# shgaurav1/DVG

Hardware: AMD Instinct MI355X
Metric: predicted frames/sec at 64x64, batch 64, 10-in/10-out (higher is better)
Workload: dtype f32; 1 GPU; Moving-MNIST 64x64 rollout (generate_frames.py make_gifs sample loop), vgg_64 + lstm + GP trigger sample at i%15==0, batch 64 per GPU, 10-in/10-out; model_family=vgg, batch_per_gpu=64, n_past=10, n_future=10, parallelism=replicas x1 (no data-path collective), launch=hipGraph replay, rollouts_in_flight=3, tile_policy=energy, loop_invariant_skip_halves=hoisted, upsample_conv3x3=as transposed 4x4/s2 conv, conv3x3_deep_layers=Winograd F(4x4,3x3) / F(2x2,3x3)

## Files before the change

dvg_amd/_lib.py:

```python
from __future__ import annotations

import ctypes as C
import os
import threading

_HERE = os.path.dirname(os.path.abspath(__file__))
LIB_PATH = os.environ.get("DVG_HIP_LIB") or os.path.join(_HERE, "csrc", "libdvg_hip.so")

_p = C.c_void_p
_i = C.c_int
_f = C.c_float
_d = C.c_double
_l = C.c_long
_ip = C.POINTER(C.c_int)

SIGNATURES = {
    "dvg_abi_version": (_i, []),
    "dvg_last_error": (C.c_char_p, []),
    "dvg_stream_capture_id": (_l, [_p]),
    "dvg_mfma_mode": (_i, []),
    "dvg_build_info": (C.c_char_p, []),
    "dvg_set_tile_policy": (None, [_i]),
    "dvg_tile_policy": (_i, []),
    "dvg_packed_row_floats": (_i, []),
    "dvg_pack_conv_weight": (_i, [_p, _p, _i, _i, _i, _i, _p]),
    "dvg_pack_convT_weight": (_i, [_p, _p, _i, _i, _i, _i, _p]),
    "dvg_unpack_conv_weight": (_i, [_p, _p, _i, _i, _i, _i, _p]),
    "dvg_unpack_convT_weight": (_i, [_p, _p, _i, _i, _i, _i, _p]),
    "dvg_conv_first_stats_rows": (_i, [_i, _i, _i, _i]),
    "dvg_pack_conv_weight_k16": (_i, [_p, _p, _i, _i, _i, _i, _i, _p]),
    "dvg_conv_splitk_v2": (_i, [_i, _i, _i, _i, _i, _i]),
    "dvg_conv_stats_rows_v2": (_i, [_i, _i, _i, _i, _i, _i, _i, _i]),
    "dvg_conv3x3_bn_act_v2": (_i, [_p, _p, _p, _p, _p, _p, _p, _p, _i, _i, _i, _i, _i, _i, _i, _i, _f, _p, _l, _p, _p, _i, _p]),
    "dvg_conv3x3_first_pair": (_i, [_p, _p, _p, _p, _p, _p, _p, _p, _p, _i, _i, _i, _i, _i, _f, _i, _p]),
    "dvg_conv4x4s2_bn_act_v2": (_i, [_p, _p, _p, _p, _p, _p, _i, _i, _i, _i, _i, _i, _f, _p, _l, _p]),
    "dvg_convT4x4s2_bn_act_v2": (_i, [_p, _p, _p, _p, _p, _p, _p, _i, _i, _i, _i, _i, _i, _i, _f, _p, _l, _p, _p, _i, _p]),
    "dvg_convT4x4s2_bn_act_proj": (_i, [_p, _p, _p, _p, _p, _p, _i, _i, _i, _i, _i, _i, _i, _f, _p, _p, _i, _p]),
    "dvg_winograd_weight": (_i, [_p, _p, _i, _i, _i, _p]),
    "dvg_winograd_input": (_i, [_p, _p, _i, _i, _i, _i, _i, _i, _p]),
    "dvg_gemm_batched_k16": (_i, [_p, _p, _p, _i, _i, _i, _i, _i, _p]),
    "dvg_gemm_batched_plan": (_i, [_i, _i, _i, _i, _i, _ip, _ip, _ip]),
    "dvg_winograd_transform_width": (_i, [_l, _i]),
    "dvg_winograd_output": (_i, [_p, _p, _p, _p, _p, _i, _i, _i, _i, _i, _f, _i, _p, _i, _p]),
    "dvg_winograd_output_input": (_i, [_p, _p, _p, _p, _i, _i, _i, _i, _i, _f, _p, _p]),
    "dvg_stem_up_winograd_input": (_i, [_p, _i, _p, _i, _p, _p, _p, _i, _i, _i, _i, _f, _p]),
    "dvg_winograd_output_up_input": (_i, [_p, _p, _p, _p, _i, _i, _i, _i, _i, _f, _p]),
    "dvg_winograd_output_pool_input": (_i, [_p, _p, _p, _p, _p, _i, _i, _i, _i, _i, _f, _i, _p]),
    "dvg_conv3x3_first": (_i, [_p, _p, _p, _p, _p, _p, _i, _i, _i, _i, _i, _i, _f, _p]),
    "dvg_convT3x3_last": (_i, [_p, _p, _p, _p, _i, _i, _i, _i, _i, _i, _p]),
    "dvg_conv4x4s2_first": (_i, [_p, _p, _p, _p, _p, _p, _i, _i, _i, _i, _i, _i, _f, _p]),
    "dvg_convT4x4s2_last": (_i, [_p, _p, _p, _p, _p, _i, _i, _i, _i, _i, _i, _i, _p]),
    "dvg_moving_mnist_compose": (_i, [_p, _p, _p, _p, _i, _i, _i, _i, _i, _i, _p]),
    "dvg_clip_gather_u8": (_i, [_p, _p, _p, _l, _i, _i, _i, _i, _i, _i, _p]),
    "dvg_clip_gather_aug_u8": (_i, [_p, _p, _p, _p, _p, _l, _i, _i, _i, _i, _i, _i, _p]),
    "dvg_mnist_scale_u8": (_i, [_p, _p, _i, _i, _i, _p, _p, _p]),
    "dvg_moving_mnist_compose_u8": (_i, [_p, _p, _p, _p, _i, _i, _i, _i, _i, _i, _p]),
    "dvg_resample_u8_band": (_i, [_p, _i, _i, _i, _i, _i, _i, _p]),
    "dvg_resample_u8": (_i, [_p, _p, _i, _i, _i, _i, _i, _i, _p, _p, _i, _p, _p, _i, _p, _p]),
    "dvg_eval_frames": (_i, [_p, _p, _p, _p, _i, _i, _i, _p]),
    "dvg_eval_frames_finn": (_i, [_p, _p, _p, _p, _p, _i, _i, _i, _i, _p]),
    "dvg_pairwise_frame_mse": (_i, [_p, _p, _i, _l, _i, _l, _i, _p]),
    "dvg_frame_mosaic": (_i, [_p, _l, _p, _l, _p, _l, _i, _i, _i, _p] + [_i] * 9 + [_p, _i, _p, _i, _i, _p, _i, _i, _i, _i, _p, _p]),
    "dvg_adam_step": (_i, [_p, _p, _p, _p, _l, _f, _f, _f, _f, _f, _i, _p, _p]),
    "dvg_pixel_proj": (_i, [_p, _p, _p, _l, _i, _i, _p]),
    "dvg_convT_gather": (_i, [_p, _p, _p, _p, _i, _i, _i, _i, _i, _i, _p, _i, _p]),
    "dvg_channel_stats_rows": (_i, [_l]),
    "dvg_channel_stats": (_i, [_p, _p, _l, _i, _i, _p]),
    "dvg_bn_finalize": (_i, [_p, _i, _p, _p, _p, _p, _p, _p, _p, _p, _i, _d, _f, _f, _p, _i, _i, _p, _p]),
    "dvg_channel_stats_pivot": (_i, [_p, _p, _p, _l, _i, _i, _p]),
    "dvg_bn_finalize_pivot": (_i, [_p, _i, _p, _p, _p, _p, _p, _p, _p, _p, _p, _i, _d, _f, _f, _p, _i, _i, _p, _p]),
    "dvg_bn_running_update": (_i, [_p, _p, _i, _i, _f, _f, _f, _p, _p, _p, _i, _p]),
    "dvg_bn_act_apply": (_i, [_p, _p, _p, _p, _p, _i, _i, _i, _i, _i, _f, _i, _p]),
    "dvg_gemm_nt_bias_act": (_i, [_p, _p, _p, _p, _p, _p, _i, _i, _i, _i, _i, _i, _i, _i, _f, _i, _p]),
    "dvg_lstm_cell": (_i, [_p, _p, _p, _p, _p, _p, _p, _p, _p, _p, _i, _i, _p]),
    "dvg_lstm_cell_pre": (_i, [_p, _p, _p, _p, _p, _p, _p, _i, _i, _p]),
    "dvg_lstm_cell_bwd": (_i, [_p, _p, _p, _p, _p, _p, _p, _p, _p, _p, _i, _i, _p]),
    "dvg_lstm_cell_x": (_i, [_p, _i, _i, _p, _p, _p, _i, _p, _p, _p, _p, _i, _i, _p]),
    "dvg_gru_cell": (_i, [_p, _p, _p, _p, _p, _p, _p, _p, _i, _i, _p]),
    "dvg_gru_cell_pre": (_i, [_p, _p, _p, _p, _p, _p, _i, _i, _p]),
    "dvg_rnn_cell": (_i, [_p, _p, _p, _p, _p, _p, _p, _i, _i, _p]),
    "dvg_gru_gates_bwd": (_i, [_p, _p, _p, _p, _p, _p, _p, _i, _i, _p]),
    "dvg_stem_gemm": (_i, [_p, _i, _p, _i, _p, _p, _p, _i, _i, _i, _i, _i, _i, _f, _p]),
    "dvg_gp_precision": (_i, [_i, _i, _i]),
    "dvg_gp_bwd_precision": (_i, [_i, _i]),
    "dvg_gp_lds_bytes": (C.c_size_t, [_i, _i, _i]),
    "dvg_gp_predict": (_i, [_p] * 14 + [_i, _i, _i, _i, _f, _i, _i, _p]),
    "dvg_gp_step_group": (_i, [_i, _i, _i, _i]),
    "dvg_gp_bwd_lds_bytes": (C.c_size_t, [_i, _i]),
    "dvg_gp_bwd_chunk": (_i, [_i, _i]),
    "dvg_gemm_tn": (_i, [_p] * 5 + [_i] * 8 + [_p]),
    "dvg_gp_train_bwd": (_i, [_p] * 17 + [_i, _i, _i, _f, _i, _i, _p]),
    "dvg_sum_steps_multi": (_i, [_p, _p, _p, _i, _i, _p]),
    "dvg_gp_elbo": (_i, [_p, _p, _p, _p, _l, _l, _p, _p, _i, _i, _i, _i, _p]),
    "dvg_gp_elbo_bwd": (_i, [_p, _p, _p, _p, _l, _l, _p, _p, _p, _p, _p, _p, _p, _i, _i, _i, _i, _p]),
    "dvg_bn_act_bwd_rows": (_i, [_i, _i, _i, _i]),
    "dvg_bn_act_bwd_reduce": (_i, [_p, _p, _p, _p, _p, _p, _i, _i, _i, _i, _i, _f, _i, _p]),
    "dvg_bn_bwd_finalize": (_i, [_p, _i, _p, _p, _p, _p, _p, _p, _p, _p, _p, _i, _d, _i, _i, _i, _p]),
    "dvg_bn_act_bwd_reduce_centered": (_i, [_p, _p, _p, _p, _p, _p, _p, _i, _i, _i, _i, _i, _f, _i, _p]),
    "dvg_bn_bwd_finalize_centered": (_i, [_p, _i, _p, _p, _p, _p, _p, _p, _p, _p, _p, _i, _d, _i, _i, _i, _p]),
    "dvg_affine3_apply": (_i, [_p, _p, _p, _p, _p, _p, _l, _i, _p, _i, _i, _p]),
    "dvg_act_bwd": (_i, [_p, _p, _p, _l, _i, _f, _p]),
    "dvg_upsample2x_bwd": (_i, [_p, _p, _i, _i, _i, _i, _p]),
    "dvg_group_sum": (_i, [_p, _p, _p, _i, _i, _l, _p]),
    "dvg_colsum": (_i, [_p, _p, _i, _i, _i, _p]),
    "dvg_wgrad_finish": (_i, [_p, _i, _p, _i, _i, _i, _i, _i, _i, _i, _f, _p]),
    "dvg_k4_to_w3": (_i, [_p, _p, _i, _i, _i, _i, _f, _p]),
    "dvg_reduce_partials": (_i, [_p, _p, _i, _l, _p]),
    "dvg_conv_wgrad_splits": (_i, [_i, _i, _i, _i, _i, _i]),
    "dvg_conv_wgrad": (_i, [_i, _p, _p, _p, _p, _i, _i, _i, _i, _i, _i, _i, _p]),
    "dvg_conv_wgrad_splits_multi": (_i, [_i, _i, _i, _i, _i, _i, _i]),
    "dvg_conv_wgrad_multi": (_i, [_i, _i, _p, _p, _p, _p, _i, _i, _i, _i, _i, _i, _i, _p]),
    "dvg_winograd_wgrad_operands": (_i, [_p, _p, _p, _p, _i, _i, _i, _i, _i, _l, _l, _p]),
    "dvg_winograd_wgrad_splits": (_i, [_l, _i, _i]),
    "dvg_winograd_wgrad_gemm": (_i, [_p, _p, _p, _l, _i, _i, _p]),
    "dvg_winograd_wgrad_gemm_items": (_i, [_p, _p, _i, _l, _p, _i, _i, _p]),
    "dvg_winograd_wgrad_reduce": (_i, [_p, _i, _p, _i, _i, _p]),
    "dvg_wgrad_thin_rows": (_i, [_i, _i, _i, _i]),
    "dvg_wgrad_thin": (_i, [_p, _p, _p, _i, _i, _i, _i, _i, _i, _p]),
    "dvg_lstm_gates_bwd": (_i, [_p, _p, _p, _p, _p, _p, _p, _i, _i, _p]),
    "dvg_nchw_to_nhwc": (_i, [_p, _p, _i, _i, _i, _i, _p]),
    "dvg_nhwc_to_nchw": (_i, [_p, _p, _i, _i, _i, _i, _p]),
    "dvg_zero_tick": (_i, [_p, _l, _p, _p, _p, _p, _p]),
    "dvg_grad_sumsq_blocks": (_i, [_l]),
    "dvg_grad_sumsq": (_i, [_p, _l, _p, _p]),
    "dvg_grad_guard_finish": (_i, [_p, _i, _d, _i, _p, _p, _p]),
    "dvg_adam_step_guarded": (_i, [_p, _p, _p, _p, _l, _f, _f, _f, _f, _f, _i, _p, _p, _p, _p]),
    "dvg_ema_update_blocks": (_i, [_l]),
    "dvg_ema_update": (_i, [_p, _p, _l, _d, _p, _p, _p]),
    "dvg_lr_schedule_tick": (_i, [_i, _i, _i, _i, _d, _d, _p, _p, _p]),
    "dvg_adam_step_scheduled": (_i, [_p, _p, _p, _p, _l, _f, _f, _f, _f, _f, _i, _p, _p, _p, _p, _p]),
    "dvg_optim_step": (_i, [_i, _p, _p, _p, _p, _l, _f, _f, _f, _f, _f, _i, _p, _i, _p, _p, _p, _p, _p]),
    "dvg_val_accumulate": (_i, [_p, _p, _p, _i, _i, _i, _p, _p, _p, _p]),
    "dvg_frame_losses_blocks": (_i, [_l]),
    "dvg_frame_losses": (_i, [_p, _p, _p, _p, _l, _i, _i, _p, _p, _p]),
    "dvg_mse_sum_grad": (_i, [_p, _p, _p, _p, _l, _f, _p]),
    "dvg_frame_losses_ext_blocks": (_i, [_i, _l, _i, _i]),
    "dvg_frame_losses_ext": (_i, [_p, _p, _p, _p, _i, _i, _l, _i, _i, _i, _f, _p, _p, _p, _p]),
    "dvg_frame_ssim_loss_blocks": (_i, [_i, _l, _i, _i]),
    "dvg_frame_ssim_loss": (_i, [_p, _p, _p, _p, _i, _i, _l, _i, _i, _p, _i, _p, _p]),
    "dvg_gp_var_norms": (_i, [_p, _p, _i, _i, _p]),
    "dvg_gp_trigger_step": (_i, [_p, _i, _i, _i, _p, _i, _f, _p, _p, _p, _p, _i, _p]),
    "dvg_gp_trigger_replay": (_i, [_p, _i, _p, _i, _f, _p, _p, _p]),
    "dvg_gp_trigger_select": (_i, [_p, _p, _p, _p, _i, _i, _i, _l, _p, _p, _p, _p]),
    "dvg_debug_set_clockbuf": (None, [_p, C.c_uint]),
    "dvg_debug_set_gp_clockbuf": (None, [_p, C.c_uint]),
    "dvg_debug_set_wgrad_clockbuf": (None, [_p, C.c_uint]),
}

_lock = threading.Lock()
_lib = None


class DvgLibraryError(RuntimeError):
    pass


def lib() -> C.CDLL:
    global _lib
    if _lib is not None:
        return _lib
    with _lock:
        if _lib is not None:
            return _lib
        if not os.path.exists(LIB_PATH):
            raise DvgLibraryError(
                f"{LIB_PATH} not found: the HIP kernel library has not been built. "
                "Run `python -c 'import __graft_entry__ as g; g.build()'` (or `make -C dvg_amd/csrc`). "
                "There is no CPU/eager fallback for the DVG hot path.")
        try:
            import torch
            if torch.cuda.is_available():
                torch.cuda.init()
        except ImportError:
            pass
        try:
            handle = C.CDLL(LIB_PATH)
        except OSError as e:
            raise DvgLibraryError(f"cannot load {LIB_PATH}: {e}") from e
        for name, (res, args) in SIGNATURES.items():
            try:
                fn = getattr(handle, name)
            except AttributeError as e:
                raise DvgLibraryError(f"{LIB_PATH} lacks symbol {name}; rebuild it") from e
            fn.restype = res
            fn.argtypes = args
        _lib = handle
        return _lib


def build_info() -> dict:
    raw = lib().dvg_build_info().decode()
    d = {}
    for tok in raw.split():
        k, _, v = tok.partition("=")
        d[k] = int(v) if v.lstrip("-").isdigit() else v
# ... 13 lines not shown
```

dvg_amd/csrc/winograd.hip:

```cpp
#include <cstdlib>

#include "dvg_common.h"

namespace dvg {

__global__ void winograd_weight_kernel(const float* __restrict__ w, float* __restrict__ u, int cout, int cin) {
    const unsigned total = (unsigned)cout * (unsigned)cin / 2;
    for (unsigned i = blockIdx.x * blockDim.x + threadIdx.x; i < total; i += gridDim.x * blockDim.x) {
        const unsigned rr = i >> 3;
        const int co = (int)(rr % (unsigned)cout), chunk = (int)(rr / (unsigned)cout), k = (int)(i & 7) * 2;
        const float* g = w + ((size_t)co * cin + chunk * 16 + k) * 9;
        float t[2][4][3];
#pragma unroll
        for (int e = 0; e < 2; ++e)
#pragma unroll
            for (int s = 0; s < 3; ++s) {
                const float g0 = g[9 * e + s], g1 = g[9 * e + 3 + s], g2 = g[9 * e + 6 + s];
                t[e][0][s] = g0;
                t[e][1][s] = 0.5f * (g0 + g1 + g2);
                t[e][2][s] = 0.5f * (g0 - g1 + g2);
                t[e][3][s] = g2;
            }
        const unsigned row0 = ((unsigned)(co >> 6) * (unsigned)(cin / 16) + (unsigned)chunk) * 64u + (unsigned)(co & 63);
        const unsigned pos_rows = (unsigned)(cout >> 6) * (unsigned)(cin / 16) * 64u;
// ... 342 lines not shown
            for (int qq = 0; qq < 4; ++qq) {
                const float ad = addend ? addend[(((size_t)n * HW + 4 * ty + pp) * HW + 4 * tx + qq) * C + c] : 0.f;
                ys[((4 * ty + pp) * HW + 4 * tx + qq) * CS + cl] = apply_act((o[qq] + ad) * sc + sf, act, slope);
            }
        }
    }
    __syncthreads();
    float e[6][6];
#pragma unroll
    for (int b = 0; b < 6; ++b) {
        const int xx = 4 * tx - 1 + b;
        float d[6];
#pragma unroll
        for (int a = 0; a < 6; ++a) {
            const int yy = 4 * ty - 1 + a;
            d[a] = ((unsigned)yy < (unsigned)HW && (unsigned)xx < (unsigned)HW) ? ys[(yy * HW + xx) * CS + cl] : 0.f;
        }
        float col[6];
        bt4(d, col);
#pragma unroll
        for (int a = 0; a < 6; ++a) e[a][b] = col[a];
    }
#pragma unroll
    for (int a = 0; a < 6; ++a) {
        float o[6];
        bt4(e[a], o);
#pragma unroll
        for (int b = 0; b < 6; ++b) v[((size_t)(a * 6 + b) * T + t) * C + c] = o[b];
    }
}

template <int HW, int CS, typename V, bool POOL, int NT, bool UP = false>
__global__ __launch_bounds__(NT) void winograd4_chain_kernel(const float* __restrict__ m, const float* __restrict__ scale,
                                                             const float* __restrict__ shift, float* __restrict__ y,
                                                             float* __restrict__ v, int N, int C, int act, float slope,
                                                             const float* __restrict__ addend, int y_from) {
    constexpr int VN = VecN<V>::N;
    constexpr int WT = HW / 4, TI = WT * WT;
    static_assert(!(POOL && UP), "pool and upsample exclude each other");
    constexpr int SS = POOL ? HW / 2 : HW;
    constexpr int S2 = UP ? 2 * HW : SS;
    constexpr int WT2 = S2 / 4, TI2 = WT2 * WT2;
    constexpr int CV = CS / VN;
    extern __shared__ __attribute__((aligned(16))) float chain_ys[];
    float* const ys = chain_ys;
    const int cblocks = C / CS;
    const int n = blockIdx.x / cblocks, c0 = (blockIdx.x % cblocks) * CS;
    const int CVg = C / VN;
    const long T = (long)N * TI;
    for (int u = threadIdx.x; u < TI * CV; u += NT) {
        const int cv = u % CV, t_img = u / CV, ty = t_img / WT, tx = t_img % WT;
        const long t = (long)n * TI + t_img;
        const int cg = c0 / VN + cv;
        V s[4][6];
#pragma unroll
        for (int b = 0; b < 6; ++b) {
            V q[6];
#pragma unroll
            for (int a = 0; a < 6; ++a) q[a] = __builtin_nontemporal_load(reinterpret_cast<const V*>(m) + ((size_t)(a * 6 + b) * T + t) * CVg + cg);
            V col[4];
            at4(q, col);
#pragma unroll
            for (int pp = 0; pp < 4; ++pp) s[pp][b] = col[pp];
        }
        V sc, sf;
#pragma unroll
        for (int k = 0; k < VN; ++k) {
            vset(sc, k, scale ? scale[c0 + cv * VN + k] : 1.f);
            vset(sf, k, shift ? shift[c0 + cv * VN + k] : 0.f);
        }
        V val[4][4];
#pragma unroll
        for (int pp = 0; pp < 4; ++pp) {
            V o[4];
            at4(s[pp], o);
#pragma unroll
            for (int qq = 0; qq < 4; ++qq) {
                V ad = vzero<V>();
                if (addend) ad = reinterpret_cast<const V*>(addend)[(((size_t)n * HW + 4 * ty + pp) * HW + 4 * tx + qq) * CVg + cg];
#pragma unroll
                for (int k = 0; k < VN; ++k)
                    vset(val[pp][qq], k, apply_act((vget(o[qq], k) + vget(ad, k)) * vget(sc, k) + vget(sf, k), act, slope));
                if (POOL) {
                    if (n >= y_from)
                        reinterpret_cast<V*>(y)[(((size_t)(n - y_from) * HW + 4 * ty + pp) * HW + 4 * tx + qq) * CVg + cg] = val[pp][qq];
                } else
                    *reinterpret_cast<V*>(&ys[((4 * ty + pp) * HW + 4 * tx + qq) * CS + cv * VN]) = val[pp][qq];
            }
        }
        if (POOL) {
#pragma unroll
            for (int pp = 0; pp < 2; ++pp)
#pragma unroll
                for (int qq = 0; qq < 2; ++qq) {
                    V mx;
#pragma unroll
                    for (int k = 0; k < VN; ++k)
                        vset(mx, k, fmaxf(fmaxf(vget(val[2 * pp][2 * qq], k), vget(val[2 * pp][2 * qq + 1], k)),
                                          fmaxf(vget(val[2 * pp + 1][2 * qq], k), vget(val[2 * pp + 1][2 * qq + 1], k))));
                    *reinterpret_cast<V*>(&ys[((2 * ty + pp) * SS + 2 * tx + qq) * CS + cv * VN]) = mx;
                }
        }
    }
    __syncthreads();
    const long T2 = (long)N * TI2;
    for (int u = threadIdx.x; u < TI2 * CV; u += NT) {
        const int cv = u % CV, t_img = u / CV, ty = t_img / WT2, tx = t_img % WT2;
        const long t2 = (long)n * TI2 + t_img;
        const int cg = c0 / VN + cv;
        V e[6][6];
#pragma unroll
        for (int b = 0; b < 6; ++b) {
            const int xx = 4 * tx - 1 + b;
            V d[6];
#pragma unroll
            for (int a = 0; a < 6; ++a) {
                const int yy = 4 * ty - 1 + a;
                d[a] = ((unsigned)yy < (unsigned)S2 && (unsigned)xx < (unsigned)S2)
                           ? *reinterpret_cast<const V*>(&ys[((yy >> (UP ? 1 : 0)) * SS + (xx >> (UP ? 1 : 0))) * CS + cv * VN])
                           : vzero<V>();
            }
            V col[6];
            bt4(d, col);
#pragma unroll
            for (int a = 0; a < 6; ++a) e[a][b] = col[a];
        }
#pragma unroll
        for (int a = 0; a < 6; ++a) {
            V o[6];
            bt4(e[a], o);
#pragma unroll
            for (int b = 0; b < 6; ++b) reinterpret_cast<V*>(v)[((size_t)(a * 6 + b) * T2 + t2) * CVg + cg] = o[b];
        }
    }
}

template <int HW, int CS, typename V, bool POOL, int NT, bool UP = false>
static int launch_chain(const float* mm, const float* scale, const float* shift, float* y, float* v, int N, int C, int act,
                        float slope, hipStream_t st, const float* addend = nullptr, int y_from = 0) {
    constexpr int S2 = POOL ? HW / 2 : HW;
    constexpr size_t lds = (size_t)S2 * S2 * CS * 4;
    auto kern = winograd4_chain_kernel<HW, CS, V, POOL, NT, UP>;
    static bool attr = false;
    if (!attr && lds > 48 * 1024) {
        hipError_t e = hipFuncSetAttribute(reinterpret_cast<const void*>(kern), hipFuncAttributeMaxDynamicSharedMemorySize, (int)lds);
        if (e != hipSuccess) return fail(DVG_ERR_HIP, "hipFuncSetAttribute: %s", hipGetErrorString(e));
        attr = true;
    }
    hipLaunchKernelGGL(kern, dim3((unsigned)((long)N * (C / CS))), dim3(NT), lds, st, mm, scale, shift, y, v, N, C, act, slope,
                       addend, y_from);
    return check_launch("winograd4_chain");
}

template <int KP>
__global__ __launch_bounds__(256) void stem_up_input_kernel(const float* __restrict__ vec, int ldv, const float* __restrict__ wt,
                                                            const float* __restrict__ scale, const float* __restrict__ shift,
                                                            float* __restrict__ v, int M, int C, int K, int act, float slope) {
    constexpr int BR = 8;
    __shared__ float vs[BR * KP];
    __shared__ float ys[BR * 16 * 16];
    const int tid = threadIdx.x, cl = tid & 15, hw = tid >> 4;
    const int c = blockIdx.x * 16 + cl;
    const size_t N = (size_t)16 * C, n = (size_t)hw * C + c;
    const int m0 = blockIdx.y * BR, mrows = min(BR, M - m0);
    for (int i = tid; i < BR * KP; i += 256) {
        const int r = i / KP, k = i % KP;
        vs[i] = (r < mrows && k < K) ? vec[(size_t)(m0 + r) * ldv + k] : 0.f;
    }
    float w[KP];
#pragma unroll
    for (int k = 0; k < KP; ++k) w[k] = wt[(size_t)k * N + n];
    __syncthreads();
    const float sc = scale ? scale[c] : 1.f, sf = shift ? shift[c] : 0.f;
#pragma unroll
    for (int bb = 0; bb < BR; ++bb) {
        const f32x4* vr = reinterpret_cast<const f32x4*>(vs + bb * KP);
        float s0 = 0.f, s1 = 0.f;
#pragma unroll
        for (int k4 = 0; k4 < KP / 4; ++k4) {
            const f32x4 v4 = vr[k4];
            s0 = fmaf(v4[0], w[4 * k4], s0);
            s1 = fmaf(v4[1], w[4 * k4 + 1], s1);
            s0 = fmaf(v4[2], w[4 * k4 + 2], s0);
            s1 = fmaf(v4[3], w[4 * k4 + 3], s1);
        }
        ys[(bb * 16 + hw) * 16 + cl] = apply_act((s0 + s1) * sc + sf, act, slope);
    }
    __syncthreads();
    const long T = (long)M * 4;
    for (int u = tid; u < BR * 64; u += 256) {
        const int ucl = u & 15, tile = (u >> 4) & 3, bb = u >> 6;
        if (bb >= mrows) continue;
        const int ty = tile >> 1, tx = tile & 1;
        const float* src = ys + bb * 256 + ucl;
        float e[6][6];
#pragma unroll
        for (int b = 0; b < 6; ++b) {
            const int xx = 4 * tx - 1 + b;
            float d[6];
#pragma unroll
            for (int a = 0; a < 6; ++a) {
                const int yy = 4 * ty - 1 + a;
                d[a] = ((unsigned)yy < 8u && (unsigned)xx < 8u) ? src[((yy >> 1) * 4 + (xx >> 1)) * 16] : 0.f;
            }
            float col[6];
            bt4(d, col);
#pragma unroll
            for (int a = 0; a < 6; ++a) e[a][b] = col[a];
        }
        const long t = (long)(m0 + bb) * 4 + tile;
        float* dst = v + t * C + blockIdx.x * 16 + ucl;
#pragma unroll
        for (int a = 0; a < 6; ++a) {
            float o[6];
            bt4(e[a], o);
#pragma unroll
            for (int b = 0; b < 6; ++b) dst[(size_t)(a * 6 + b) * T * C] = o[b];
        }
    }
}

static int wino4_width(long tiles, int C) {
    if (tiles * (C / 4) >= 1024L * 256) return 4;
    if (tiles * (C / 2) >= 1024L * 256) return 2;
    return 1;
}

static int chain_variant() { return 0; }

static inline unsigned wgrid(long n) {
    long g = (n + 255) / 256;
    return (unsigned)(g > 16384 ? 16384 : (g < 1 ? 1 : g));
}

}

using namespace dvg;

extern "C" int dvg_winograd_weight(const float* w_oihw, float* u_k16, int cout, int cin, int m, void* stream) {
    DVG_REQUIRE(w_oihw && u_k16, DVG_ERR_NULL, "dvg_winograd_weight: NULL pointer");
    DVG_REQUIRE(cout > 0 && cout % 64 == 0 && cin > 0 && cin % 16 == 0 && (m == 2 || m == 4), DVG_ERR_SHAPE,
                "dvg_winograd_weight: Cin must be a multiple of 16, Cout of 64, m 2 or 4");
    if (m == 2)
        hipLaunchKernelGGL(winograd_weight_kernel, dim3(wgrid((long)cout * cin / 2)), dim3(256), 0, (hipStream_t)stream, w_oihw,
                           u_k16, cout, cin);
    else
        hipLaunchKernelGGL(winograd4_weight_kernel, dim3(wgrid((long)cout * cin / 2)), dim3(256), 0, (hipStream_t)stream, w_oihw,
                           u_k16, cout, cin);
    return check_launch("dvg_winograd_weight");
}

extern "C" int dvg_winograd_input(const float* x, float* v, int N, int H, int W, int C, int m, int upsample, void* stream) {
    DVG_REQUIRE(x && v, DVG_ERR_NULL, "dvg_winograd_input: NULL pointer");
    DVG_REQUIRE((m == 2 || m == 4) && N > 0 && H > 0 && W > 0 && H % m == 0 && W % m == 0 && C > 0 && C % 4 == 0,
                DVG_ERR_SHAPE, "dvg_winograd_input: m 2 or 4, H and W multiples of m, C %% 4 == 0 needed");
    DVG_REQUIRE(upsample == 0 || (upsample == 1 && m == 4 && H % 2 == 0 && W % 2 == 0), DVG_ERR_SHAPE,
                "dvg_winograd_input: upsample needs m = 4 and even H, W");
    const int up = upsample;
    DVG_REQUIRE(aligned16(x) && aligned16(v), DVG_ERR_ALIGN, "dvg_winograd_input: alignment");
    const long tiles = (long)N * (H / m) * (W / m);
    const hipStream_t st = (hipStream_t)stream;
    if (m == 2) {
        hipLaunchKernelGGL(winograd_input_kernel, dim3(wgrid(tiles * (C / 4))), dim3(256), 0, st, x, v, N, H, W, C / 4);
    } else {
        const int cw = wino4_width(tiles, C);
        if (cw == 4)
            hipLaunchKernelGGL(winograd4_input_kernel<f32x4>, dim3(wgrid(tiles * (C / 4))), dim3(256), 0, st, x, v, N, H, W, C / 4, tiles, 0L, up);
        else if (cw == 2)
            hipLaunchKernelGGL(winograd4_input_kernel<f32x2>, dim3(wgrid(tiles * (C / 2))), dim3(256), 0, st, x, v, N, H, W, C / 2, tiles, 0L, up);
        else
            hipLaunchKernelGGL(winograd4_input_kernel<float>, dim3(wgrid(tiles * C)), dim3(256), 0, st, x, v, N, H, W, C, tiles, 0L, up);
    }
    return check_launch("dvg_winograd_input");
}

extern "C" int dvg_winograd_transform_width(long tiles, int C) {
    if (tiles <= 0 || C <= 0 || C % 4) return 0;
    return wino4_width(tiles, C);
}

extern "C" int dvg_winograd_wgrad_operands(const float* x, const float* dy, float* v, float* dm, int N, int H, int W, int Cin,
                                           int Cout, long t_total, long t_off, void* stream) {
    DVG_REQUIRE((x && v) || (dy && dm), DVG_ERR_NULL, "dvg_winograd_wgrad_operands: nothing to do");
    DVG_REQUIRE(N > 0 && H > 0 && W > 0 && H % 4 == 0 && W % 4 == 0 && Cin > 0 && Cin % 4 == 0 && Cout > 0 && Cout % 4 == 0,
                DVG_ERR_SHAPE, "dvg_winograd_wgrad_operands: H and W multiples of 4, channels multiples of 4 needed");
    const long tiles = (long)N * (H / 4) * (W / 4);
    DVG_REQUIRE(t_off >= 0 && t_off + tiles <= t_total, DVG_ERR_SHAPE,
                "dvg_winograd_wgrad_operands: tiles [%ld, %ld) outside the buffer of %ld", t_off, t_off + tiles, t_total);
    DVG_REQUIRE(aligned16(x) && aligned16(dy) && aligned16(v) && aligned16(dm), DVG_ERR_ALIGN,
                "dvg_winograd_wgrad_operands: alignment");
    const hipStream_t st = (hipStream_t)stream;
#define WOPS(KERNEL_, SRC_, DST_, C_, ...)                                                                                        \
    do {                                                                                                                       \
        const int cw_ = wino4_width(tiles, (C_));                                                                              \
        if (cw_ == 4)                                                                                                          \
            hipLaunchKernelGGL(KERNEL_<f32x4>, dim3(wgrid(tiles * ((C_) / 4))), dim3(256), 0, st, SRC_, DST_, N, H, W, (C_) / 4, t_total, t_off __VA_ARGS__); \
        else if (cw_ == 2)                                                                                                     \
            hipLaunchKernelGGL(KERNEL_<f32x2>, dim3(wgrid(tiles * ((C_) / 2))), dim3(256), 0, st, SRC_, DST_, N, H, W, (C_) / 2, t_total, t_off __VA_ARGS__); \
        else                                                                                                                   \
            hipLaunchKernelGGL(KERNEL_<float>, dim3(wgrid(tiles * (C_))), dim3(256), 0, st, SRC_, DST_, N, H, W, (C_), t_total, t_off __VA_ARGS__);           \
    } while (0)
    if (x && v) {
        WOPS(winograd4_input_kernel, x, v, Cin, , 0);
        if (int e = check_launch("dvg_winograd_wgrad_operands (input)")) return e;
    }
    if (dy && dm) {
        WOPS(winograd4_dy_kernel, dy, dm, Cout, );
        if (int e = check_launch("dvg_winograd_wgrad_operands (dy)")) return e;
    }
#undef WOPS
    return DVG_OK;
}

extern "C" int dvg_winograd_output_input(const float* mm, const float* scale, const float* shift, float* v_next, int N, int H,
                                         int W, int C, int act, float slope, const float* addend, void* stream) {
    DVG_REQUIRE(mm && v_next, DVG_ERR_NULL, "dvg_winograd_output_input: NULL pointer");
    DVG_REQUIRE(aligned16(addend), DVG_ERR_ALIGN, "dvg_winograd_output_input: addend alignment");
    DVG_REQUIRE(N > 0 && H == W && (H == 8 || H == 16 || H == 32) && C > 0 && C % 64 == 0, DVG_ERR_SHAPE,
                "dvg_winograd_output_input: 8x8, 16x16 or 32x32 maps, C %% 64 == 0 needed (got %dx%d, C=%d)", H, W, C);
    DVG_REQUIRE(act >= 0 && act <= 3, DVG_ERR_SHAPE, "dvg_winograd_output_input: bad act");
    DVG_REQUIRE(aligned16(mm) && aligned16(v_next), DVG_ERR_ALIGN, "dvg_winograd_output_input: alignment");
    const hipStream_t st = (hipStream_t)stream;
    const int var = chain_variant();
    if (H == 8) {
        hipLaunchKernelGGL(winograd4_out_in_kernel<8>, dim3((unsigned)((long)N * (C / 64))), dim3(256), 0, st, mm, scale, shift,
                           v_next, N, C, act, slope, addend);
    } else if (H == 16) {
        if (var == 9) {
            hipLaunchKernelGGL(winograd4_out_in_kernel<16>, dim3((unsigned)((long)N * (C / 16))), dim3(256), 0, st, mm, scale,
                               shift, v_next, N, C, act, slope, addend);
        } else if (var == 2 || (var == 0 && (long)N * (C / 64) < 1024)) {
            return launch_chain<16, 32, float, false, 512>(mm, scale, shift, nullptr, v_next, N, C, act, slope, st, addend);
        } else {
            return launch_chain<16, 64, f32x2, false, 512>(mm, scale, shift, nullptr, v_next, N, C, act, slope, st, addend);
        }
    } else {
        if (var == 1) return launch_chain<32, 16, f32x2, false, 512>(mm, scale, shift, nullptr, v_next, N, C, act, slope, st, addend);
        return launch_chain<32, 32, f32x4, false, 512>(mm, scale, shift, nullptr, v_next, N, C, act, slope, st, addend);
    }
    return check_launch("dvg_winograd_output_input");
}

extern "C" int dvg_stem_up_winograd_input(const float* vec, int ldv, const float* w_kn, int KP, const float* scale,
                                          const float* shift, float* v_next, int M, int C, int K, int act, float slope,
                                          void* stream) {
    DVG_REQUIRE(vec && w_kn && v_next, DVG_ERR_NULL, "dvg_stem_up_winograd_input: NULL pointer");
    DVG_REQUIRE(M > 0 && C > 0 && C % 16 == 0 && K > 0 && K <= KP && (KP == 96 || KP == 128) && ldv >= K, DVG_ERR_SHAPE,
                "dvg_stem_up_winograd_input: bad shape M=%d C=%d K=%d KP=%d (C %% 16 == 0, KP 96 or 128)", M, C, K, KP);
    DVG_REQUIRE(act >= 0 && act <= 3, DVG_ERR_SHAPE, "dvg_stem_up_winograd_input: bad act");
    DVG_REQUIRE(aligned16(v_next), DVG_ERR_ALIGN, "dvg_stem_up_winograd_input: alignment");
    const dim3 grid(C / 16, (M + 7) / 8);
    if (KP == 96)
        hipLaunchKernelGGL(stem_up_input_kernel<96>, grid, dim3(256), 0, (hipStream_t)stream, vec, ldv, w_kn, scale, shift, v_next,
                           M, C, K, act, slope);
    else
        hipLaunchKernelGGL(stem_up_input_kernel<128>, grid, dim3(256), 0, (hipStream_t)stream, vec, ldv, w_kn, scale, shift, v_next,
                           M, C, K, act, slope);
    return check_launch("dvg_stem_up_winograd_input");
}

extern "C" int dvg_winograd_output_up_input(const float* mm, const float* scale, const float* shift, float* v_next, int N, int H,
                                            int W, int C, int act, float slope, void* stream) {
    DVG_REQUIRE(mm && v_next, DVG_ERR_NULL, "dvg_winograd_output_up_input: NULL pointer");
    DVG_REQUIRE(N > 0 && H == W && H == 8 && C > 0 && C % 64 == 0, DVG_ERR_SHAPE,
                "dvg_winograd_output_up_input: 8x8 maps, C %% 64 == 0 needed (got %dx%d, C=%d)", H, W, C);
    DVG_REQUIRE(act >= 0 && act <= 3, DVG_ERR_SHAPE, "dvg_winograd_output_up_input: bad act");
    DVG_REQUIRE(aligned16(mm) && aligned16(v_next), DVG_ERR_ALIGN, "dvg_winograd_output_up_input: alignment");
    const hipStream_t st = (hipStream_t)stream;
    return launch_chain<8, 32, float, false, 512, true>(mm, scale, shift, nullptr, v_next, N, C, act, slope, st);
}

extern "C" int dvg_winograd_output_pool_input(const float* mm, const float* scale, const float* shift, float* y, float* v_next,
                                              int N, int H, int W, int C, int act, float slope, int y_from, void* stream) {
    DVG_REQUIRE(mm && v_next && (y || y_from == N), DVG_ERR_NULL, "dvg_winograd_output_pool_input: NULL pointer");
    DVG_REQUIRE(y_from >= 0 && y_from <= N, DVG_ERR_SHAPE, "dvg_winograd_output_pool_input: y_from=%d outside [0, N]", y_from);
    DVG_REQUIRE(N > 0 && H == W && (H == 16 || H == 32) && C > 0 && C % 64 == 0, DVG_ERR_SHAPE,
                "dvg_winograd_output_pool_input: 16x16 or 32x32 maps, C %% 64 == 0 needed (got %dx%d, C=%d)", H, W, C);
    DVG_REQUIRE(act >= 0 && act <= 3, DVG_ERR_SHAPE, "dvg_winograd_output_pool_input: bad act");
    DVG_REQUIRE(aligned16(mm) && aligned16(y) && aligned16(v_next), DVG_ERR_ALIGN, "dvg_winograd_output_pool_input: alignment");
    const hipStream_t st = (hipStream_t)stream;
    const int var = chain_variant();
    (void)var;
    if (H == 16) return launch_chain<16, 64, f32x2, true, 512>(mm, scale, shift, y, v_next, N, C, act, slope, st, nullptr, y_from);
    return launch_chain<32, 32, f32x2, true, 1024>(mm, scale, shift, y, v_next, N, C, act, slope, st, nullptr, y_from);
}

extern "C" int dvg_winograd_output(const float* m, const float* scale, const float* shift, float* y, float* y_pool, int N,
                                   int H, int W, int C, int act, float slope, int mt, const float* addend, int y_from,
                                   void* stream) {
    DVG_REQUIRE(m && (y || (y_pool && y_from == N)), DVG_ERR_NULL, "dvg_winograd_output: NULL pointer");
    DVG_REQUIRE(y_from >= 0 && y_from <= N && (y_from == 0 || y_pool != nullptr), DVG_ERR_SHAPE,
                "dvg_winograd_output: y_from=%d needs 0 <= y_from <= N and a pooled output", y_from);
    DVG_REQUIRE(addend == nullptr || (mt == 4 && y_pool == nullptr && aligned16(addend)), DVG_ERR_SHAPE,
                "dvg_winograd_output: addend needs m = 4, no pooled output, 16-byte alignment");
    DVG_REQUIRE((mt == 2 || mt == 4) && N > 0 && H > 0 && W > 0 && H % mt == 0 && W % mt == 0 && C > 0 && C % 4 == 0,
                DVG_ERR_SHAPE, "dvg_winograd_output: m 2 or 4, H and W multiples of m, C %% 4 == 0 needed");
    DVG_REQUIRE(act >= 0 && act <= 3, DVG_ERR_SHAPE, "dvg_winograd_output: bad act");
    DVG_REQUIRE(aligned16(m) && aligned16(y) && aligned16(y_pool) && aligned16(scale) && aligned16(shift), DVG_ERR_ALIGN,
                "dvg_winograd_output: alignment");
    const unsigned g = wgrid((long)N * (H / mt) * (W / mt) * (C / 4));
    const hipStream_t st = (hipStream_t)stream;
    if (mt == 2 && y_pool)
        hipLaunchKernelGGL(winograd_output_kernel<true>, dim3(g), dim3(256), 0, st, m, scale, shift, y, y_pool, N, H, W, C / 4, act, slope, y_from);
    else if (mt == 2)
        hipLaunchKernelGGL(winograd_output_kernel<false>, dim3(g), dim3(256), 0, st, m, scale, shift, y, y_pool, N, H, W, C / 4, act, slope, 0);
    else {
        const long tiles = (long)N * (H / 4) * (W / 4);
#define W4OUT(POOL_, V_, CW_)                                                                                             \
    hipLaunchKernelGGL((winograd4_output_kernel<POOL_, V_>), dim3(wgrid(tiles * (C / CW_))), dim3(256), 0, st, m, scale, shift, \
                       y, y_pool, N, H, W, C / CW_, act, slope, addend, y_from)
        const int cw = wino4_width(tiles, C);
        if (cw == 4) { if (y_pool) W4OUT(true, f32x4, 4); else W4OUT(false, f32x4, 4); }
        else if (cw == 2) { if (y_pool) W4OUT(true, f32x2, 2); else W4OUT(false, f32x2, 2); }
        else { if (y_pool) W4OUT(true, float, 1); else W4OUT(false, float, 1); }
#undef W4OUT
    }
    return check_launch("dvg_winograd_output");
}
```

include/dvg_hip.h:

```cpp
#ifndef DVG_HIP_H
#define DVG_HIP_H

#include <stddef.h>
#include <stdint.h>

#ifdef __cplusplus
extern "C" {
#endif

#define DVG_OK 0
#define DVG_ERR_SHAPE 1
#define DVG_ERR_NULL 2
#define DVG_ERR_HIP 3
#define DVG_ERR_ALIGN 4

#define DVG_ACT_NONE 0
#define DVG_ACT_LRELU 1
#define DVG_ACT_TANH 2
#define DVG_ACT_SIGMOID 3

int dvg_abi_version(void);
const char* dvg_last_error(void);
long dvg_stream_capture_id(void* stream);

int dvg_pack_conv_weight(const float* w_oihw, float* w_packed, int cout, int cin, int kh, int kw, void* stream);

int dvg_pack_convT_weight(const float* w_iohw, float* w_packed, int cin, int cout, int kh, int kw, void* stream);

int dvg_unpack_conv_weight(const float* w_packed, float* w_oihw, int cout, int cin, int kh, int kw, void* stream);
int dvg_unpack_convT_weight(const float* w_packed, float* w_iohw, int cin, int cout, int kh, int kw, void* stream);

#define DVG_MODE_CONV3 0
#define DVG_MODE_CONV4S2 1
#define DVG_MODE_CONVT4S2 2
int dvg_conv_first_stats_rows(int ks, int N, int H, int W);

int dvg_mfma_mode(void);
int dvg_packed_row_floats(void);
const char* dvg_build_info(void);
void dvg_set_tile_policy(int energy);
int dvg_tile_policy(void);
int dvg_pack_conv_weight_k16(const float* w, float* w_packed, int cout, int cin, int kh, int kw, int transposed, void* stream);
int dvg_conv_splitk_v2(int mode, int N, int H, int W, int Cin, int Cout);
int dvg_conv_stats_rows_v2(int mode, int N, int H, int W, int Cin, int Cout, int pool, int with_workspace);
int dvg_conv3x3_bn_act_v2(const float* x, const float* skip, const float* w_k16, const float* scale, const float* shift, float* y,
                          float* y_pool, float* stats, int N, int H, int W, int C1, int C2, int Cout, int upsample_x, int act,
                          float slope, float* workspace, long workspace_floats, const float* addend,
                          const int* addend_map, int addend_block, void* stream);
int dvg_conv3x3_first_pair(const float* frame, const float* w0, const float* scale0, const float* shift0,
                           const float* w1_k16, const float* scale1, const float* shift1, float* y, float* y_pool,
                           int N, int H, int W, int Cout, int act, float slope,
                           int y_from ,
                           void* stream);
int dvg_conv4x4s2_bn_act_v2(const float* x, const float* w_k16, const float* scale, const float* shift, float* y, float* stats,
                            int N, int H, int W, int Cin, int Cout, int act, float slope, float* workspace, long workspace_floats,
                            void* stream);
int dvg_convT4x4s2_bn_act_v2(const float* x, const float* skip, const float* w_k16, const float* scale, const float* shift, float* y,
                             float* stats, int N, int H, int W, int C1, int C2, int Cout, int act, float slope, float* workspace,
                             long workspace_floats, const float* addend, const int* addend_map , int addend_block, void* stream);
int dvg_convT4x4s2_bn_act_proj(const float* x, const float* w_k16, const float* scale, const float* shift, const float* proj_w, float* proj_out, int T,
                               int N, int H, int W, int C1, int Cout, int act, float slope, const float* addend, const int* addend_map, int addend_block, void* stream);

int dvg_winograd_weight(const float* w_oihw, float* u_k16, int cout, int cin, int m, void* stream);
int dvg_winograd_input(const float* x, float* v, int N, int H, int W, int C, int m, int upsample, void* stream);
int dvg_gemm_batched_k16(const float* x, const float* w_k16, float* y, int NB, int H, int W, int Cin, int Cout, void* stream);
int dvg_gemm_batched_plan(int NB, int H, int W, int Cin, int Cout, int* tile_w, int* nt, int* ni);
int dvg_winograd_transform_width(long tiles, int C);
int dvg_winograd_output(const float* mm, const float* scale, const float* shift, float* y, float* y_pool, int N, int H,
                        int W, int C, int act, float slope, int m, const float* addend,
                        int y_from , void* stream);
int dvg_winograd_output_input(const float* mm, const float* scale, const float* shift, float* v_next, int N, int H, int W,
                              int C, int act, float slope, const float* addend , void* stream);
int dvg_stem_up_winograd_input(const float* vec, int ldv, const float* w_kn, int KP, const float* scale, const float* shift,
                               float* v_next, int M, int C, int K, int act, float slope, void* stream);
int dvg_winograd_output_up_input(const float* mm, const float* scale, const float* shift, float* v_next, int N, int H, int W,
                                 int C, int act, float slope, void* stream);
int dvg_winograd_output_pool_input(const float* m, const float* scale, const float* shift, float* y, float* v_next, int N,
                                   int H, int W, int C, int act, float slope, int y_from, void* stream);

int dvg_conv3x3_first(const float* x_nchw, const float* w_oihw, const float* scale, const float* shift, float* y, float* stats,
                      int N, int H, int W, int nc, int Cout, int act, float slope, void* stream);

int dvg_convT3x3_last(const float* x, const float* w_iohw, const float* bias, float* y_nchw, int N, int H, int W, int Cin,
                      int nc, int act, void* stream);

int dvg_conv4x4s2_first(const float* x_nchw, const float* w_oihw, const float* scale, const float* shift, float* y, float* stats,
                        int N, int H, int W, int nc, int Cout, int act, float slope, void* stream);

int dvg_convT4x4s2_last(const float* x, const float* skip, const float* w_iohw, const float* bias, float* y_nchw, int N, int H,
                        int W, int C1, int C2, int nc, int act, void* stream);

int dvg_pixel_proj(const float* in, const float* w, float* out, long P, int C, int T, void* stream);

int dvg_convT_gather(const float* d1, const float* d2, const float* bias, float* y_nchw, int ks,
                     int N, int H, int W, int nc, int act,
                     const int* d2_map ,
                     int d2_block, void* stream);


int dvg_channel_stats_rows(long rows);
int dvg_channel_stats(const float* u, float* stats_partial, long rows, int C, int groups, void* stream);
int dvg_channel_stats_pivot(const float* u, float* stats_partial, const float* pivot, long rows, int C, int groups,
                            void* stream);

int dvg_bn_finalize(const float* stats_partial, int nrows, const float* gamma,
                    const float* beta, float* scale, float* shift, float* running_mean,
                    float* running_var, float* save_mean, float* save_invstd,
                    int C, double count, float eps, float momentum,
                    int64_t* num_batches_tracked , int nbt_inc, int groups,
                    float* group_var, void* stream);
int dvg_bn_finalize_pivot(const float* stats_partial, int nrows, const float* pivot, const float* gamma,
                          const float* beta, float* scale, float* shift, float* running_mean, float* running_var,
                          float* save_mean, float* save_invstd, int C, double count, float eps, float momentum,
                          int64_t* num_batches_tracked, int nbt_inc, int groups, float* group_var, void* stream);
int dvg_bn_running_update(const float* mean, const float* unbiased_var, int groups, int C, float mom_first, float mom_mid,
                          float mom_last, float* running_mean, float* running_var, int64_t* num_batches_tracked,
                          int nbt_inc, void* stream);

int dvg_bn_act_apply(const float* u, const float* scale, const float* shift, float* y,
                     float* y_pool, int N, int H, int W, int C, int act, float slope,
                     int group_images, void* stream);

int dvg_gemm_nt_bias_act(const float* a, const float* w, const float* scale, const float* shift, float* out, float* workspace,
                         int M, int N, int K, int lda, int ldo, int period, int splitk, int act, float slope,
                         int accumulate , void* stream);

int dvg_lstm_cell(const float* x, const float* h, const float* c, const float* w_ih, const float* w_hh, const float* b_ih,
                  const float* b_hh, float* h_out, float* c_out, float* gates_out, int B, int H, void* stream);

int dvg_lstm_cell_pre(const float* pre, const float* h, const float* c, const float* w_hh, float* h_out,
                      float* c_out, float* gates_out, int B, int H, void* stream);
int dvg_lstm_cell_bwd(const float* dh_a, const float* dh_b, const float* dc, const float* gates,
                      const float* c_prev, const float* c_new, const float* w_hh_t, float* dG, float* dc_prev,
                      float* dh_prev, int B, int H, void* stream);

int dvg_lstm_cell_x(const float* x, int ldx, int Kx, const float* h, const float* c, const float* w_x, int Kxp,
                    const float* w_hh, const float* bias, float* h_out, float* c_out, int B, int H, void* stream);

int dvg_gru_cell(const float* x, const float* h, const float* w_ih, const float* w_hh, const float* b_ih, const float* b_hh,
                 float* h_out, float* acts_out, int B, int H, void* stream);
int dvg_gru_cell_pre(const float* pre, const float* h, const float* w_hh, const float* b_hn, float* h_out, float* acts_out,
                     int B, int H, void* stream);
int dvg_rnn_cell(const float* x, const float* h, const float* w_ih, const float* w_hh, const float* b_ih, const float* b_hh,
                 float* h_out, int B, int H, void* stream);
int dvg_gru_gates_bwd(const float* dh_a, const float* dh_b, const float* acts, const float* h_prev, float* dGi, float* dGh,
                      float* dh_prev, int B, int H, void* stream);

int dvg_stem_gemm(const float* vec, int ldv, const float* w_kn, int KP, const float* scale, const float* shift,
                  float* out, int ldo, int M, int N, int K, int period, int act, float slope, void* stream);


int dvg_gp_precision(int B, int M, int need_cov);
size_t dvg_gp_lds_bytes(int B, int M, int need_cov);
int dvg_gp_predict(const float* h, const float* z, const float* var_mean, const float* chol_var, const float* mean_const,
                   const float* outputscale, const float* lengthscale, const float* noise, const float* eps, float* mean,
                   float* var, float* sample, float* cov, float* kl, int B, int D, int M, int train_mode, float jitter,
                   int param_period ,
                   int step_group ,
                   void* stream);
int dvg_gp_step_group(int B, int S, int P, int M);


int dvg_bn_act_bwd_rows(int N, int H, int W, int pool);
int dvg_bn_act_bwd_reduce(const float* dy, const float* dyp, const float* y, const float* u,
                          float* dp, float* partial, int N, int H, int W, int C, int act,
                          float slope, int groups, void* stream);
int dvg_bn_act_bwd_reduce_centered(const float* dy, const float* dyp, const float* y, const float* u, const float* mean,
                                   float* dp, float* partial, int N, int H, int W, int C, int act, float slope,
                                   int groups, void* stream);
int dvg_bn_bwd_finalize(const float* partial, int nrows, const float* gamma, const float* mean,
                        const float* invstd, float* coefA, float* coefB, float* coefC,
                        float* dgamma, float* dbeta, float* dbias, int C, double count,
                        int train, int accumulate , int groups, void* stream);
int dvg_bn_bwd_finalize_centered(const float* partial, int nrows, const float* gamma, const float* mean,
                                 const float* invstd, float* coefA, float* coefB, float* coefC,
                                 float* dgamma, float* dbeta, float* dbias, int C, double count,
                                 int train, int accumulate, int groups, void* stream);
int dvg_affine3_apply(const float* dp, const float* u, const float* A, const float* B,
                      const float* Cc, float* du, long n, int C, float* sum, int sum_mode,
                      int groups , void* stream);
int dvg_group_sum(const float* src, const int* map, float* dst, int groups, int blocks, long block_elems, void* stream);
int dvg_act_bwd(const float* dy, const float* y, float* dpre, long n, int act, float slope,
                void* stream);
int dvg_upsample2x_bwd(const float* dxu, float* dx, int N, int H, int W, int C, void* stream);
int dvg_colsum(const float* a, float* out, int rows, int C, int accumulate , void* stream);
int dvg_reduce_partials(const float* partial, float* out, int S, long n, void* stream);

int dvg_conv_wgrad_splits(int mode, int N, int H, int W, int Cin, int Cout);
int dvg_conv_wgrad(int mode, const float* x, const float* skip, const float* dout,
                   float* partial, int N, int H, int W, int C1, int C2, int Cout,
                   int upsample_x, void* stream);
int dvg_conv_wgrad_splits_multi(int mode, int N, int H, int W, int Cin, int Cout, int items);
int dvg_conv_wgrad_multi(int mode, int items, const float* const* x, const float* const* skip,
                         const float* const* dout, float* partial, int N, int H, int W, int C1, int C2,
                         int Cout, int upsample_x, void* stream);

int dvg_winograd_wgrad_operands(const float* x, const float* dy, float* v, float* dm, int N, int H, int W, int Cin,
                                int Cout, long t_total, long t_off, void* stream);
int dvg_winograd_wgrad_splits(long t_total, int Cin, int Cout);
int dvg_winograd_wgrad_gemm(const float* dm, const float* v, float* partial, long t_total, int Cin, int Cout, void* stream);
int dvg_winograd_wgrad_gemm_items(const float* dm, const float* const* v_items, int items, long tiles_per_item,
                                  float* partial, int Cin, int Cout, void* stream);
int dvg_winograd_wgrad_reduce(const float* partial, int S, float* packed, int Cin, int Cout, void* stream);

int dvg_wgrad_finish(const float* partial, int S, float* dst, int kind, int kh, int kw, int cout, int cin, int ctot,
                     int c_lo, float beta, void* stream);
int dvg_k4_to_w3(const float* dk4_packed, float* dw, int cout, int c1, int ctot, int c_lo, float beta, void* stream);

int dvg_wgrad_thin_rows(int ks, int N, int Hi, int Wi);
int dvg_wgrad_thin(const float* inp_nchw, const float* dout_nhwc, float* partial, int ks, int N, int Hi, int Wi, int nc, int C, void* stream);

int dvg_moving_mnist_compose(const float* sprites, const int* ids, const int* pos, float* out, int n_sprites, int T, int B, int num_digits, int image_size, int digit_size, void* stream);

int dvg_clip_gather_u8(const uint8_t* pool, const int64_t* first, float* out, int64_t n_frames, int T, int B, int C, int H, int W, int pool_c, void* stream);
int dvg_clip_gather_aug_u8(const uint8_t* pool, const int64_t* first, const int32_t* geom, const float* photo, float* out, int64_t n_frames, int T, int B, int C, int H, int W, int pool_c, void* stream);

int dvg_mnist_scale_u8(const uint8_t* raw, uint8_t* out, int n, int in_size, int out_size, const int* xmin, const int* coef, void* stream);
int dvg_resample_u8_band(const int* ymin_host, int Hin, int Win, int Hout, int Wout, int C, int yk, int* span);
int dvg_resample_u8(const uint8_t* src, uint8_t* dst, int n, int Hin, int Win, int Hout, int Wout, int C, const int* xmin, const int* xcoef, int xk, const int* ymin, const int* ycoef, int yk, const int* ymin_host, void* stream);

// ... 98 lines not shown
```

Measured before the change: 52890 frames/s.

## Stage Winograd F(4x4) input bands in LDS for 32-wide 64/128-channel layers

Adds a Winograd F(4x4,3x3) input-transform kernel that loads a band of input rows (with halo) into LDS using 16-byte vector loads and an XOR-swizzled column layout, then computes the 6x6 tile transforms from LDS. It is selected for W=32, C=64 or 128, when the existing width heuristic would not pick the widest vector path, and it also covers the upsample case. The goal is to avoid re-reading overlapping 6x6 tile windows from global memory and to make the loads coalesced. In exchange it uses large LDS allocations per block, which may lower occupancy, and adds a query entry point for the chosen form.

```diff
diff --git a/dvg_amd/_lib.py b/dvg_amd/_lib.py
--- a/dvg_amd/_lib.py
+++ b/dvg_amd/_lib.py
@@ -41,6 +41,7 @@
     "dvg_gemm_batched_k16": (_i, [_p, _p, _p, _i, _i, _i, _i, _i, _p]),
     "dvg_gemm_batched_plan": (_i, [_i, _i, _i, _i, _i, _ip, _ip, _ip]),
     "dvg_winograd_transform_width": (_i, [_l, _i]),
+    "dvg_winograd_input_form": (_i, [_i, _i, _i, _i, _i, _i]),
     "dvg_winograd_output": (_i, [_p, _p, _p, _p, _p, _i, _i, _i, _i, _i, _f, _i, _p, _i, _p]),
     "dvg_winograd_output_input": (_i, [_p, _p, _p, _p, _i, _i, _i, _i, _i, _f, _p, _p]),
     "dvg_stem_up_winograd_input": (_i, [_p, _i, _p, _i, _p, _p, _p, _i, _i, _i, _i, _f, _p]),
diff --git a/dvg_amd/csrc/winograd.hip b/dvg_amd/csrc/winograd.hip
--- a/dvg_amd/csrc/winograd.hip
+++ b/dvg_amd/csrc/winograd.hip
@@ -518,6 +518,84 @@
     return check_launch("winograd4_chain");
 }
 
+template <int SH> __device__ __forceinline__ int lds_col(int x) { return x ^ ((x >> SH) & 1); }
+
+template <typename V, int WD, int CS, int R, int NT, bool UP>
+struct InputStaged {
+    static constexpr int VN = VecN<V>::N, CV = CS / VN, WT = WD / 4, WS = UP ? WD / 2 : WD;
+    static constexpr int ROWS = UP ? 2 * R + 2 : 4 * R + 2;
+    static constexpr int ROW_F4 = WS * CS / 4;
+    static constexpr size_t LDS = (size_t)ROWS * WS * CS * 4;
+};
+
+template <typename V, int WD, int CS, int R, int NT, bool UP>
+__global__ __launch_bounds__(NT) void winograd4_input_staged_kernel(const float* __restrict__ x, float* __restrict__ v, int N,
+                                                                    int H, int C) {
+    using K = InputStaged<V, WD, CS, R, NT, UP>;
+    constexpr int VN = K::VN, CV = K::CV, WT = K::WT, WS = K::WS, SH = UP ? 1 : 2, U = UP ? 1 : 0;
+    extern __shared__ __attribute__((aligned(16))) float in_ys[];
+    float* const ys = in_ys;
+    const int Ht = H >> 2, Hs = H >> U, bands = (Ht + R - 1) / R, cblocks = C / CS;
+    const int cb = blockIdx.x % cblocks, band = (blockIdx.x / cblocks) % bands, n = blockIdx.x / (cblocks * bands);
+    const int c0 = cb * CS, ty0 = band * R, rb = min(R, Ht - ty0);
+    const int s0 = max(4 * ty0 - 1, 0) >> U, s1 = min(4 * (ty0 + rb), H - 1) >> U, nrows = s1 - s0 + 1;
+    const f32x4* const src = reinterpret_cast<const f32x4*>(x + ((size_t)n * Hs + s0) * WS * C + c0);
+#pragma unroll
+    for (int i0 = 0; i0 < K::ROWS * K::ROW_F4; i0 += NT) {
+        const int i = i0 + threadIdx.x, c4 = i % (CS / 4), p = i / (CS / 4), xs = p % WS, r = p / WS;
+        if (r < nrows)
+            *reinterpret_cast<f32x4*>(&ys[(r * WS + lds_col<SH>(xs)) * CS + 4 * c4]) = src[((size_t)r * WS + xs) * (C / 4) + c4];
+    }
+    __syncthreads();
+    const int CVg = C / VN;
+    const long T = (long)N * Ht * WT;
+    for (int u = threadIdx.x; u < rb * WT * CV; u += NT) {
+        const int cv = u % CV, t_band = u / CV, tx = t_band % WT, ty = ty0 + t_band / WT;
+        const long t = ((long)n * Ht + ty) * WT + tx;
+        const int cg = c0 / VN + cv;
+        V e[6][6];
+#pragma unroll
+        for (int b = 0; b < 6; ++b) {
+            const int xx = 4 * tx - 1 + b;
+            V d[6];
+#pragma unroll
+            for (int a = 0; a < 6; ++a) {
+                const int yy = 4 * ty - 1 + a;
+                d[a] = ((unsigned)yy < (unsigned)H && (unsigned)xx < (unsigned)WD)
+                           ? *reinterpret_cast<const V*>(&ys[(((yy >> U) - s0) * WS + lds_col<SH>(xx >> U)) * CS + cv * VN])
+                           : vzero<V>();
+            }
+            V col[6];
+            bt4(d, col);
+#pragma unroll
+            for (int a = 0; a < 6; ++a) e[a][b] = col[a];
+        }
+#pragma unroll
+        for (int a = 0; a < 6; ++a) {
+            V o[6];
+            bt4(e[a], o);
+#pragma unroll
+            for (int b = 0; b < 6; ++b) reinterpret_cast<V*>(v)[((size_t)(a * 6 + b) * T + t) * CVg + cg] = o[b];
+        }
+    }
+}
+
+template <typename V, int WD, int CS, int R, int NT, bool UP>
+static int launch_input_staged(const float* x, float* v, int N, int H, int C, hipStream_t st) {
+    using K = InputStaged<V, WD, CS, R, NT, UP>;
+    static_assert(K::LDS <= 160 * 1024 && CS % 4 == 0 && K::WS % 2 == 0, "staged band must fit the LDS");
+    auto kern = winograd4_input_staged_kernel<V, WD, CS, R, NT, UP>;
+    static bool attr = false;
+    if (!attr && K::LDS > 48 * 1024) {
+        hipError_t e = hipFuncSetAttribute(reinterpret_cast<const void*>(kern), hipFuncAttributeMaxDynamicSharedMemorySize, (int)K::LDS);
+        if (e != hipSuccess) return fail(DVG_ERR_HIP, "hipFuncSetAttribute: %s", hipGetErrorString(e));
+        attr = true;
+    }
+    const int bands = ((H >> 2) + R - 1) / R;
+    hipLaunchKernelGGL(kern, dim3((unsigned)((long)N * bands * (C / CS))), dim3(NT), K::LDS, st, x, v, N, H, C);
+    return check_launch("winograd4_input_staged");
+}
+
 template <int KP>
 __global__ __launch_bounds__(256) void stem_up_input_kernel(const float* __restrict__ vec, int ldv, const float* __restrict__ wt,
                                                             const float* __restrict__ scale, const float* __restrict__ shift,
@@ -592,6 +670,10 @@
     return 1;
 }
 
+static int wino4_input_form(long tiles, int H, int W, int C, int m) {
+    return m == 4 && W == 32 && H % 4 == 0 && (C == 64 || C == 128) && wino4_width(tiles, C) < 4;
+}
+
 static int chain_variant() { return 0; }
 
 static inline unsigned wgrid(long n) {
@@ -628,6 +710,9 @@
     const hipStream_t st = (hipStream_t)stream;
     if (m == 2) {
         hipLaunchKernelGGL(winograd_input_kernel, dim3(wgrid(tiles * (C / 4))), dim3(256), 0, st, x, v, N, H, W, C / 4);
+    } else if (wino4_input_form(tiles, H, W, C, m)) {
+        if (up) return launch_input_staged<f32x2, 32, 32, 2, 256, true>(x, v, N, H, C, st);
+        return launch_input_staged<f32x2, 32, 32, 2, 256, false>(x, v, N, H, C, st);
     } else {
         const int cw = wino4_width(tiles, C);
         if (cw == 4)
@@ -638,6 +723,12 @@
             hipLaunchKernelGGL(winograd4_input_kernel<float>, dim3(wgrid(tiles * C)), dim3(256), 0, st, x, v, N, H, W, C, tiles, 0L, up);
     }
     return check_launch("dvg_winograd_input");
+}
+
+extern "C" int dvg_winograd_input_form(int N, int H, int W, int C, int m, int upsample) {
+    if (!((m == 2 || m == 4) && N > 0 && H > 0 && W > 0 && H % m == 0 && W % m == 0 && C > 0 && C % 4 == 0)) return -1;
+    if (!(upsample == 0 || (upsample == 1 && m == 4 && H % 2 == 0 && W % 2 == 0))) return -1;
+    return wino4_input_form((long)N * (H / m) * (W / m), H, W, C, m);
 }
 
 extern "C" int dvg_winograd_transform_width(long tiles, int C) {
diff --git a/include/dvg_hip.h b/include/dvg_hip.h
--- a/include/dvg_hip.h
+++ b/include/dvg_hip.h
@@ -66,6 +66,7 @@
 int dvg_gemm_batched_k16(const float* x, const float* w_k16, float* y, int NB, int H, int W, int Cin, int Cout, void* stream);
 int dvg_gemm_batched_plan(int NB, int H, int W, int Cin, int Cout, int* tile_w, int* nt, int* ni);
 int dvg_winograd_transform_width(long tiles, int C);
+int dvg_winograd_input_form(int N, int H, int W, int C, int m, int upsample);
 int dvg_winograd_output(const float* mm, const float* scale, const float* shift, float* y, float* y_pool, int N, int H,
                         int W, int C, int act, float slope, int m, const float* addend,
                         int y_from , void* stream);
```

Result: no change. 53040 frames/s (median of 6 runs) (+0.3%).
